# S-Taichiii/diffusion-model

Hardware: AMD Instinct MI355X
Metric: denoising steps/sec (CFG, T=1000, 32x32x4 latent, B=64) (higher is better)
Workload: dtype f32 (GEMMs: fp32 operands split fp16 hi+lo on the matrix cores, fp32 accumulate); 1 GPU; config 2: UnetCondWithGeomHead CFG=3.0 denoising step, B=64, 32x32x4, T=1000; global_batch=64, T=1000, parallelism=sample-sharded x1 (no per-step collective)

## Files before the change

### diffusion-model_amd/dmx/csrc/engine.hip

```cpp
#include "dmx.h"

#include <array>
#include <cmath>
#include <cstdio>
#include <cstdlib>
#include <cstring>
#include <functional>
#include <map>
#include <memory>
#include <stdexcept>
#include <string>
#include <vector>

#include "common.h"
#include "graph_slots.h"
#include "step_mode.h"
#include "igemm.h"
#include "igemm_x3.h"
#include "kernels.h"
#include "igemm_pp.h"
#include "launch.h"
#include "igemm_halo.h"
#include "tokmlp.h"
#include "eval.h"
// ... 953 lines not shown
  const bool a_scaled = a_scale.part != nullptr;
  const ConvPlan pl = conv_plan(R, cw, kind, N, H, W, epi, seg, a_scaled);
  const bool x3 = pl.x3, wino = pl.path == CONV_WINO;
  const int bm = pl.bm, bn = pl.bn, splits = pl.splits, x1 = pl.x1 ? 1 : 0;
  if (pl.path == CONV_INPUT) {
    if (res != nullptr) throw Error(DMX_E_INTERNAL, "gemm: the direct input conv takes no residual");
    if (ash != nullptr || asl != nullptr) throw Error(DMX_E_INTERNAL, "gemm: the direct input conv reads fp32 NCHW");
  } else if (a_scaled && (!x3 || ash != nullptr || epi == EPI_STATS || gn != nullptr || R.m->prec == 2)) {
    throw Error(DMX_E_INTERNAL, "gemm: device-scaled operands only on the plain split implicit GEMM");
  }
  if (gn != nullptr && ((pl.path != CONV_HALO && !wino) || ash != nullptr || src_mode != SRC_PLAIN))
    throw Error(DMX_E_INTERNAL, "gemm: GroupNorm-on-load needs the halo / Winograd conv on a plain fp32 source");
  float* partial = splits > 1 ? R.ws.get<float>((size_t)splits * M * cw.cout) : nullptr;
  if (defer != nullptr) {
    defer->fused = pl.fused;
    defer->partial = partial;
    defer->splits = splits;
    defer->bias = cw.bias;
  }
  if (R.plan) return pl.rrows;
  IgemmParams p;
  std::memset(&p, 0, sizeof(p));
  p.src = s;
  p.H = H;
  p.W = W;
  p.M = M;
  p.taps = cw.taps;
  p.geom = cw.phases == 4 ? 2 : (cw.taps == 9 ? 1 : (cw.taps == 16 ? 3 : 0));
  p.Hin = p.geom == 3 ? 2 * H : H;
  p.Win = p.geom == 3 ? 2 * W : W;
  p.Kreal = cw.taps * cw.cin;
  p.Kpad = cw.kpad;
  p.Cout = cw.cout;
  p.Npad = cw.npad;
  p.osy = p.osx = cw.phases == 4 ? 2 : 1;
  p.Hout = H * p.osy;
  p.Wout = W * p.osx;
  p.Bw = cw.B;
  p.bias = cw.bias;
  p.out = out;
  p.res = res;
  p.rowpart = rowpart;
  p.seg = seg;
  p.ksplit = pl.ksplit;
  p.partial = partial;
  p.rgrp = pl.rgrp;
  p.nphase = cw.phases;
  p.gexact = gelu_exact_flag(R);
  if (s.C != cw.cin) throw Error(DMX_E_INTERNAL, "gemm: source channels != weight channels");
  if (x3 && cw.cin < pl.bk) throw Error(DMX_E_INTERNAL, "gemm: x3 path needs Cin >= K-step");
  if (ash != nullptr && !x3) throw Error(DMX_E_INTERNAL, "gemm: f16-plane operand needs the split GEMM");
  if (src_mode != SRC_PLAIN && src_mode != SRC_NCHW) throw Error(DMX_E_INTERNAL, "gemm: unsupported source");
  const bool slabs_to_caller = splits > 1 && pl.fused && defer != nullptr;
  if (check_args()) {
    if (src_mode == SRC_PLAIN)
      check_range(R, s.src0, (size_t)N * p.Hin * p.Win * s.C * 4, "A");
    check_range(R, ash, (size_t)N * p.Hin * p.Win * s.C * 2, "A hi");
    check_range(R, asl, (size_t)N * p.Hin * p.Win * s.C * 2, "A lo");
    check_range(R, cw.B, (size_t)cw.phases * cw.npad * cw.kpad * 4, "B");
    check_range(R, partial, (size_t)splits * M * cw.cout * 4, "partial");
    if (!slabs_to_caller)
      check_range(R, out, (size_t)N * p.Hout * p.Wout * cw.cout * 4, "out");
    check_range(R, res, (size_t)N * p.Hout * p.Wout * cw.cout * 4, "res");
  }
  X3Params xp;
  xp.g = p;
  xp.Ash = ash;
  xp.Asl = asl;
  xp.Bh = cw.Bh;
  xp.Bl = cw.Bl;
  xp.inv_scale = cw.inv_scale;
  xp.Fh = cw.Fh;
  xp.Fl = cw.Fl;
  xp.gn_rowpart = nullptr;
  xp.gn_cnt = 0;
  xp.gn_gamma = xp.gn_beta = nullptr;
  xp.gn_res = nullptr;
  xp.Uh = xp.Ul = nullptr;
  xp.u_bytes = 0;
  xp.a_amax = a_scale.part;
  xp.a_nparts = a_scale.n;
  xp.w_inv = cw.inv_dev;
  {
    const size_t a_el = (size_t)N * p.Hin * p.Win * s.C;
    const size_t ab = a_el * (ash != nullptr ? 2 : 4), bb = (size_t)cw.npad * cw.kpad * 2;
    if (x3 && (ab >= ((size_t)1 << 31) || bb >= ((size_t)1 << 31)))
      throw Error(DMX_E_ARG, "gemm: operand too large for 32-bit buffer offsets (split the batch)");
    xp.a_bytes = (unsigned)ab;
    xp.b_bytes = (unsigned)bb;
  }
  const int gna = gn != nullptr ? (gn->res != nullptr ? 2 : 1) : 0;
  if (gna) {
    xp.gn_rowpart = gn->rowpart;
    xp.gn_cnt = gn->cnt;
    xp.gn_gamma = gn->gamma;
    xp.gn_beta = gn->beta;
    xp.gn_res = gn->res;
  }
  const int sa = ash != nullptr ? 1 : 0;
  const int creal = (src_mode == SRC_NCHW && s.C0) ? s.C0 : cw.cin;
  const double flops = 2.0 * (double)M * cw.phases * cw.cout * (double)cw.taps * creal;
  const double bytes = 4.0 * ((double)M * cw.phases * cw.cout + (double)N * p.Hin * p.Win * s.C +
                              (double)cw.phases * cw.cout * cw.taps * cw.cin) +
                       (splits > 1 ? 4.0 * splits * M * cw.cout : 0.0);
  const int e = splits > 1 ? (int)EPI_PARTIAL : epi;
  char nm[96];
  switch (pl.path) {
    case CONV_INPUT: {
      check_range(R, rowpart, (size_t)N * pl.rrows * (64 / 32) * sizeof(float2), "rowpart");
      ConvInParams q;
      q.x = s.src0;
      q.creal = s.C0 ? s.C0 : s.C;
      q.n_mod = s.n_mod;
      q.scale = s.scale;
      q.B = cw.B;
      q.cin = cw.cin;
      q.kpad = cw.kpad;
      q.out = out;
      q.rowpart = rowpart;
      q.H = H;
      q.W = W;
      R.begin(pl.cin_px == 32 ? "conv_in_kernel<32>" : "conv_in_kernel<16>", 2.0 * M * 64.0 * 9.0 * q.creal,
              4.0 * ((double)M * 64 + (double)M * q.creal));
      if (pl.cin_px == 32) conv_in_kernel<32><<<M / 32, 256, 0, R.st>>>(q);
      else conv_in_kernel<16><<<M / 16, 256, 0, R.st>>>(q);
      break;
    }
    case CONV_WINO:
      xp.Uh = cw.Uh;
      xp.Ul = cw.Ul;
      xp.u_bytes = (unsigned)((size_t)16 * cw.cout * s.C * 2);
      check_range(R, cw.Uh, xp.u_bytes, "U hi");
      check_range(R, cw.Ul, xp.u_bytes, "U lo");
      if (x1) std::snprintf(nm, sizeof nm, "wino_kernel<%d, %d, %d, 1>", pl.wg, gna, e);
      else std::snprintf(nm, sizeof nm, "wino_kernel<%d, %d, %d>", pl.wg, gna, e);
      R.begin(nm, flops, bytes);
      launch_wino(e, pl.wg, gna, x1, xp, dim3(wino_blocks(pl.wg, N, H), cw.cout / 64, splits), R.st);
// ... 20 lines not shown
        throw Error(DMX_E_INTERNAL, "bad epilogue");
      R.begin(nm, flops, bytes);
      if (e == EPI_PARTIAL) launch_x3_partial(bm, bn, sa, x1, xp, grid, R.st);
      else if (e == EPI_STATS) launch_x3_stats(bm, bn, sa, x1, xp, grid, R.st);
      else launch_x3_epi(e, bm, bn, sa, x1, xp, grid, R.st);
      break;
    }
    case CONV_F32: {
      const dim3 grid(cdiv(M, bm), cdiv(cw.cout, bn), splits > 1 ? splits : cw.phases);
      std::snprintf(nm, sizeof nm, "igemm_f32_kernel<%d, %d, %d, %d>", bm, bn, src_mode, e);
      if (src_mode == SRC_NCHW && e != EPI_PARTIAL && e != EPI_STATS)
        throw Error(DMX_E_INTERNAL, "bad epilogue for NCHW source");
      R.begin(nm, flops, bytes);
      launch_f32(src_mode, e, bm, bn, p, grid, R.st);
      break;
    }
  }
  R.end();
  HIPCHK(hipGetLastError());
  if (splits > 1 && !slabs_to_caller) splitk_reduce(R, pl, partial, M, cw, res, out, rowpart, seg, epi);
  return pl.rrows;
}

static void gn_finalize(Run& R, const float2* rowpart, float2* stats, int N, int rrows, int nseg, int G, int C,
                        int HWo) {
  if (R.plan) return;
  R.begin("gn_finalize_kernel", 0.0, 8.0 * (double)N * rrows * nseg);
  gn_finalize_kernel<<<N * G, 256, 0, R.st>>>(rowpart, stats, rrows, nseg, G, C, HWo, 1e-5f);
  R.end();
  HIPCHK(hipGetLastError());
}

static void norm(Run& R, NormParams np, int N) {
  if (R.plan) return;
  np.gexact = gelu_exact_flag(R);
  const int per = np.HW * (np.C / 4);
  const int target = 1024;
  const int chunks = std::max(1, std::min(cdiv(per, 256), std::max(cdiv(per, 1024), cdiv(target, N))));
  R.begin("norm_kernel", 0.0, 4.0 * (double)N * np.HW * np.C * (np.res ? 3 : 2));
  norm_kernel<<<dim3(chunks, N), 256, 0, R.st>>>(np);
  R.end();
  HIPCHK(hipGetLastError());
}

static void reduce_norm(Run& R, const Deferred& d, NormParams np, int n_src_samples) {
  if (R.plan) return;
  np.gexact = gelu_exact_flag(R);
  const int kv = std::max(RN_MIN_KV, cdiv(np.HW * (np.C / 4), 1024));
  const int n_out = np.n_src > 0 ? (np.n_fan > 0 ? np.n_fan : 2) * n_src_samples : n_src_samples;
  const int kvt = kv <= 2 ? 2 : kv <= 4 ? 4 : RN_MAXV;
  R.begin("reduce_norm_kernel<" + std::to_string(kvt) + ">", 0.0,
          4.0 * (double)n_src_samples * np.HW * np.C * (d.splits + (np.res ? 1 : 0)) +
              4.0 * (double)n_out * np.HW * np.C);
  if (kv <= 2) reduce_norm_kernel<2><<<n_src_samples, 1024, 0, R.st>>>(d.partial, d.splits, d.bias, np);
  else if (kv <= 4) reduce_norm_kernel<4><<<n_src_samples, 1024, 0, R.st>>>(d.partial, d.splits, d.bias, np);
  else reduce_norm_kernel<RN_MAXV><<<n_src_samples, 1024, 0, R.st>>>(d.partial, d.splits, d.bias, np);
  R.end();
  HIPCHK(hipGetLastError());
}

template <int SRC>
static void prep(Run& R, const SrcDesc& s, float* out, int N, int H, int W, const char* name, _Float16* oh = nullptr,
                 _Float16* ol = nullptr) {
  if (R.plan) return;
  const size_t total = (size_t)N * H * W * (s.C / 4);
  const int blocks = (int)std::min<size_t>((total + 255) / 256, 8192);
  R.begin(name, 0.0, 4.0 * (double)N * H * W * s.C * (SRC == SRC_MAXPOOL ? 5 : 2) * (oh ? 1.5 : 1.0));
  prep_kernel<SRC><<<blocks, 256, 0, R.st>>>(s, out, N, H, W, oh, ol);
  R.end();
  HIPCHK(hipGetLastError());
}

static SrcDesc plain_src(const float* p, int C) {
  SrcDesc s;
  std::memset(&s, 0, sizeof(s));
  s.src0 = p;
  s.C = C;
  s.G = 1;
  s.scale = 1.f;
  return s;
}

static NormParams norm_params(const float* raw, const float2* rowpart, int nseg, int rrows, const float* g,
                              const float* b, int C, int HW, float* out) {
  NormParams np;
  std::memset(&np, 0, sizeof(np));
  np.raw = raw;
  np.rowpart = rowpart;
  np.nseg = nseg;
  np.rrows = rrows;
  np.gamma = g;
  np.beta = b;
  np.C = C;
  np.G = 1;
  np.HW = HW;
  np.out = out;
  return np;
}

static float* resblock(Run& R, const ResW& w, const SrcDesc& in, int mode, int N, int H, int W, bool residual,
                       const float* emb, int emb_stride, int emb_off, int n_out = 0,
                       const _Float16* in_h = nullptr, const _Float16* in_l = nullptr, bool planes_out = false,
                       bool* wrote_planes = nullptr, GnLoad* defer_out = nullptr, const GnLoad* gn_in = nullptr) {
  const int M = N * H * W, HW = H * W;
  if (n_out <= 0) n_out = N;
  const int seg = 32;
  float* r1 = R.ws.get<float>((size_t)M * w.mid);
  float2* rp1 = R.ws.get<float2>((size_t)M * (w.mid / seg));
  const ConvPlan p2 = conv_plan(R, w.c2, CONV_SRC_PLAIN, N, H, W, EPI_STATS, seg);
  const bool planes = R.m->prec >= 1 && p2.takes_planes() && w.mid >= 64;
  float* a1 = R.ws.get<float>((size_t)M * w.mid);
  float* r2 = R.ws.get<float>((size_t)M * w.cout);
  float2* rp2 = R.ws.get<float2>((size_t)M * (w.cout / seg));
  float* out = R.ws.get<float>((size_t)n_out * HW * w.cout);
  Deferred d1, d2;
  if (gn_in != nullptr && (residual || mode != SRC_PLAIN))
    throw Error(DMX_E_INTERNAL, "resblock: a GroupNorm-on-load input needs a plain, non-residual block");
  const int rr1 = gemm(R, in, mode, N, H, W, w.c1, EPI_STATS, r1, nullptr, rp1, seg, in_h, in_l, &d1, gn_in);
  NormParams n1 = norm_params(r1, rp1, w.mid / seg, rr1, w.g1.p, w.b1.p, w.mid, HW, a1);
  n1.act = 1;
  _Float16* a1h = reinterpret_cast<_Float16*>(a1);
  _Float16* a1l = a1h + (size_t)M * w.mid;
  if (planes) {
    n1.out = nullptr;
    n1.out_h = a1h;
    n1.out_l = a1l;
  }
  const bool fuse1 = !d1.fused && !R.m->debug && p2.gn_load_pays(1) &&
                     (planes || p2.path == CONV_WINO);
  int rr2;
  if (fuse1) {
    GnLoad g;
    g.rowpart = rp1;
    g.cnt = rr1 * (w.mid / seg);
    g.gamma = w.g1.p;
    g.beta = w.b1.p;
    rr2 = gemm(R, plain_src(r1, w.mid), SRC_PLAIN, N, H, W, w.c2, EPI_STATS, r2, nullptr, rp2, seg, nullptr, nullptr,
               &d2, &g);
  } else {
    if (d1.fused) reduce_norm(R, d1, n1, N);
    else norm(R, n1, N);
    rr2 = gemm(R, plain_src(a1, w.mid), SRC_PLAIN, N, H, W, w.c2, EPI_STATS, r2, nullptr, rp2, seg,
               planes ? a1h : nullptr, planes ? a1l : nullptr, &d2);
  }
  if (defer_out != nullptr) *defer_out = GnLoad{};
  if (defer_out != nullptr && residual && mode == SRC_PLAIN && !d2.fused && emb == nullptr && n_out == N &&
      !R.m->debug) {
    defer_out->rowpart = rp2;
    defer_out->cnt = rr2 * (w.cout / seg);
    defer_out->gamma = w.g2.p;
    defer_out->beta = w.b2.p;
    defer_out->res = in.src0;
    if (wrote_planes != nullptr) *wrote_planes = false;
    return r2;
  }
  NormParams n2 = norm_params(r2, rp2, w.cout / seg, rr2, w.g2.p, w.b2.p, w.cout, HW, out);
  if (residual) {
    if (mode != SRC_PLAIN) throw Error(DMX_E_INTERNAL, "residual ResBlock needs a plain input");
    n2.res = in.src0;
  }
  n2.emb = emb;
  n2.emb_stride = emb_stride;
  n2.emb_off = emb_off;
  n2.n_src = n_out > N ? N : 0;
  n2.n_fan = n_out > N ? n_out / N : 0;
  const bool pout = planes_out && R.m->prec >= 1 && !R.m->debug && emb == nullptr && n_out == N && w.cout >= 64;
  if (wrote_planes != nullptr) *wrote_planes = pout;
  if (pout) {
    n2.out = nullptr;
    n2.out_h = reinterpret_cast<_Float16*>(out);
    n2.out_l = n2.out_h + (size_t)n_out * HW * w.cout;
  }
  if (d2.fused) reduce_norm(R, d2, n2, N);
  else norm(R, n2, n_out);
  R.tap(R.layer + ".r1", r1, (size_t)M * w.mid);
  R.tap(R.layer, out, (size_t)n_out * HW * w.cout);
  return out;
}

static void layernorm(Run& R, const float* x, float* y, const Vec& w, const Vec& b, int M, int C) {
  if (R.plan) return;
  const int blocks = cdiv(M, 4);
  R.begin("layernorm_kernel<" + std::to_string(C / 64) + ">", 0.0, 8.0 * (double)M * C);
  switch (C) {
    case 64: layernorm_kernel<1><<<blocks, 256, 0, R.st>>>(x, y, w.p, b.p, M, 1e-5f); break;
    case 128: layernorm_kernel<2><<<blocks, 256, 0, R.st>>>(x, y, w.p, b.p, M, 1e-5f); break;
    case 256: layernorm_kernel<4><<<blocks, 256, 0, R.st>>>(x, y, w.p, b.p, M, 1e-5f); break;
    default: throw Error(DMX_E_INTERNAL, "layernorm: unsupported C");
  }
  R.end();
  HIPCHK(hipGetLastError());
}

static void attention_core(Run& R, const float* qkv, float* out, int N, int L, int C, float* stats = nullptr) {
  if (R.plan) return;
  const int D = C / 4;
  if (D != 16 && D != 32 && D != 64) throw Error(DMX_E_INTERNAL, "attention: unsupported head dim");
  const bool x3 = R.m->prec >= 1 || stats != nullptr;
  if (stats != nullptr && R.m->prec == 2) throw Error(DMX_E_INTERNAL, "attention stats: not in fp16 mode");
  if (x3 && D == 16 && att16_lds_bytes(L, 0) <= 160 * 1024) {
    const int x1 = R.m->prec == 2 ? 1 : 0, nw = L > 256 ? 16 : 8;
    R.begin("attention16_kernel<" + std::to_string(nw) + ", " + std::to_string(x1) + ">", 4.0 * N * (double)L * L * C,
            4.0 * (double)N * L * 4 * C);
    HIPCHK(launch_attention16(nw, x1, qkv, out, L, C, N, R.st, stats));
    R.end();
    HIPCHK(hipGetLastError());
    return;
  }
  if (x3) {
    dim3 grid(cdiv(L, 128), 4, N);
    const int x1 = R.m->prec == 2 ? 1 : 0, wpe = D == 16 ? 4 : 1;
    R.begin("attention_x3_kernel<" + std::to_string(D) + ", " + std::to_string(wpe) + ", " + std::to_string(x1) + ">",
// ... 194 lines not shown
    SrcDesc mp = plain_src(cur, cc);
    mp.Hs = ch;
    mp.Ws = cw;
    const int nh = ch / 2, nw = cw / 2;
    const int nb = i == 0 ? S : N;
    R.layer = "down" + std::to_string(i + 1) + ".0";
    const size_t pool_el = (size_t)nb * nh * nw * cc;
    float* pooled = R.ws.get<float>(pool_el);
    const ConvPlan r0c1 = conv_plan(R, m->down[i].r0.c1, CONV_SRC_PLAIN, nb, nh, nw, EPI_STATS, 32);
    const ConvPlan r1c1 = conv_plan(R, m->down[i].r1.c1, CONV_SRC_PLAIN, nb, nh, nw, EPI_STATS, 32);
    const bool pool_planes = R.m->prec >= 1 && m->down[i].r0.c1.Bh != nullptr && !R.m->debug && !r0c1.reads_fp32();
    _Float16* pool_h = pool_planes ? R.ws.get<_Float16>(2 * pool_el) : nullptr;
    _Float16* pool_l = pool_planes ? pool_h + pool_el : nullptr;
    prep<SRC_MAXPOOL>(R, mp, pooled, nb, nh, nw, "prep_kernel<2>", pool_h, pool_l);
    bool hp = false;
    float* h0 = resblock(R, m->down[i].r0, plain_src(pooled, cc), SRC_PLAIN, nb, nh, nw, true, nullptr, 0, 0, 0,
                         pool_h, pool_l, r1c1.takes_planes(), &hp);
    R.layer = "down" + std::to_string(i + 1) + ".1";
    const _Float16* h0h = hp ? reinterpret_cast<const _Float16*>(h0) : nullptr;
    float* h1 = resblock(R, m->down[i].r1, plain_src(h0, cc), SRC_PLAIN, nb, nh, nw, false, emb, m->hsum,
                         m->down[i].emb_off, N, h0h, hp ? h0h + (size_t)nb * nh * nw * cc : nullptr);
    cc = m->down[i].cout;
    ch = nh;
    cw = nw;
    R.layer = "sa" + std::to_string(i + 1);
    cur = attn_block(R, m->sa[i], h1, N, ch, cw);
  }
  const _Float16 *cur_h = nullptr, *cur_l = nullptr;
  for (int i = 0; i < m->nbot; ++i) {
    R.layer = "bot" + std::to_string(i + 1);
    bool hp = false;
    const bool nxt = i + 1 < m->nbot &&
                     conv_plan(R, m->bot[i + 1].c1, CONV_SRC_PLAIN, N, ch, cw, EPI_STATS, 32).takes_planes();
    cur = resblock(R, m->bot[i], plain_src(cur, cc), SRC_PLAIN, N, ch, cw, false, nullptr, 0, 0, 0, cur_h, cur_l, nxt,
                   &hp);
    cc = m->bot[i].cout;
    cur_h = hp ? reinterpret_cast<const _Float16*>(cur) : nullptr;
    cur_l = hp ? cur_h + (size_t)N * ch * cw * cc : nullptr;
  }
  for (int i = 0; i < 3; ++i) {
    const int si = 2 - i;
    SrcDesc u = plain_src(skips[si], sc[si] + cc);
    u.C0 = sc[si];
    u.n_mod = si == 0 && S < N ? S : 0;
    u.src1 = cur;
    u.Hs = ch;
    u.Ws = cw;
    const int dy = sh[si] - 2 * ch, dx = sw[si] - 2 * cw;
    u.padT = dy > 0 ? dy / 2 : 0;
    u.padL = dx > 0 ? dx / 2 : 0;
    REQUIRE(u.C == m->up[i].r0.cin, "up: channel mismatch");
    R.layer = "up" + std::to_string(i + 1) + ".0";
    const size_t cat_el = (size_t)N * sh[si] * sw[si] * u.C;
    float* cat = R.ws.get<float>(cat_el);
    const ConvPlan r0c1 = conv_plan(R, m->up[i].r0.c1, CONV_SRC_PLAIN, N, sh[si], sw[si], EPI_STATS, 32);
    const ConvPlan r1c1 = conv_plan(R, m->up[i].r1.c1, CONV_SRC_PLAIN, N, sh[si], sw[si], EPI_STATS, 32);
    const bool cat_planes = R.m->prec >= 1 && m->up[i].r0.c1.Bh != nullptr && !R.m->debug && !r0c1.reads_fp32();
    _Float16* cat_h = cat_planes ? R.ws.get<_Float16>(2 * cat_el) : nullptr;
    _Float16* cat_l = cat_planes ? cat_h + cat_el : nullptr;
    prep<SRC_UPCAT>(R, u, cat, N, sh[si], sw[si], "prep_kernel<3>", cat_h, cat_l);
    bool hp = false;
    GnLoad dly;
    const bool try_defer = !R.m->debug && R.m->prec >= 1 && r1c1.gn_load_pays(2);
    float* h0 = resblock(R, m->up[i].r0, plain_src(cat, u.C), SRC_PLAIN, N, sh[si], sw[si], true, nullptr, 0, 0, 0,
                         cat_h, cat_l, r1c1.takes_planes(), &hp, try_defer ? &dly : nullptr);
    R.layer = "up" + std::to_string(i + 1) + ".1";
    const _Float16* h0h = hp ? reinterpret_cast<const _Float16*>(h0) : nullptr;
    float* h1 = dly.rowpart != nullptr
                    ? resblock(R, m->up[i].r1, plain_src(h0, u.C), SRC_PLAIN, N, sh[si], sw[si], false, emb, m->hsum,
                               m->up[i].emb_off, 0, nullptr, nullptr, false, nullptr, nullptr, &dly)
                    : resblock(R, m->up[i].r1, plain_src(h0, u.C), SRC_PLAIN, N, sh[si], sw[si], false, emb, m->hsum,
                               m->up[i].emb_off, 0, h0h, hp ? h0h + (size_t)N * sh[si] * sw[si] * u.C : nullptr);
    ch = sh[si];
    cw = sw[si];
    cc = m->up[i].cout;
    R.layer = "sa" + std::to_string(4 + i);
    cur = attn_block(R, m->sa[3 + i], h1, N, ch, cw);
  }
  return const_cast<float*>(cur);
}

static void check_shapes(dmx_model* m, int n, int h, int w) {
  if (!m->finalized) throw Error(DMX_E_STATE, "model weights not finalized");
  if (m->kind == DMX_VAE) throw Error(DMX_E_ARG, "not a U-Net model");
  REQUIRE(n >= 1, "batch must be >= 1");
  REQUIRE(h >= 8 && w >= 8, "latent must be at least 8x8");
  REQUIRE(h == w, "AttenionBlock assumes square maps (models/unet_cond.py:46-47)");
  REQUIRE(m->ctx->pos_table != nullptr, "time table not set (dmx_set_time_table)");
}

using GraphSlot = decltype(dmx_model::graphs)::Slot;

static void drop_slot(dmx_model* m, GraphSlot* s) {
  if (s->val.gexec) (void)hipGraphExecDestroy(s->val.gexec);
  if (s->val.graph) (void)hipGraphDestroy(s->val.graph);
  if (s->val.gexec_k) (void)hipGraphExecDestroy(s->val.gexec_k);
  if (s->val.graph_k) (void)hipGraphDestroy(s->val.graph_k);
  m->graphs.release(s);
}

static void drop_graph(dmx_model* m) {
  for (GraphSlot& s : m->graphs.slot) drop_slot(m, &s);
}

static void ensure_planes(dmx_model* m, hipStream_t st) {
  if (!m->planes_stale || m->prec < 1) return;
  drop_graph(m);
  for_each_conv(m, [&](ConvW& c) {
    if (c.Bh != nullptr) split_planes(c, st, m->amax);
  });
  m->planes_stale = false;
}

static bool poison_ws() {
  static const bool v = [] {
    const char* e = std::getenv("DMX_POISON");
    return e != nullptr && std::atoi(e) != 0;
  }();
// ... 835 lines not shown
```

### diffusion-model_amd/dmx/csrc/igemm_wino.h

```cpp
#pragma once
#include "common.h"
#include "igemm.h"
#include "igemm_x3.h"
#include "source.h"

namespace dmx {

#ifndef DMX_DIAG
#define DMX_DIAG 0
#endif
#if DMX_DIAG
constexpr int WSTAMP_SLOTS = 32, WSTAMP_BLOCKS = 2048;
__device__ unsigned long long g_wstamp[WSTAMP_SLOTS * WSTAMP_BLOCKS * 5];
DMX_DEV void wstamp(int slot, int k) {
  if (threadIdx.x == 0 && slot >= 0 && slot < WSTAMP_SLOTS) {
    const int b = (blockIdx.z * gridDim.y + blockIdx.y) * gridDim.x + blockIdx.x;
    if (b < WSTAMP_BLOCKS) {
      unsigned long long* q = g_wstamp + ((size_t)slot * WSTAMP_BLOCKS + b) * 5;
      q[k] = __builtin_amdgcn_s_memtime();
      if (k == 0) q[4] = ((unsigned long long)__builtin_amdgcn_s_getreg((20 << 0) | (0 << 6) | (3 << 11)) << 32) |
                         (unsigned)__builtin_amdgcn_s_getreg((4 << 0) | (0 << 6) | (31 << 11));
    }
  }
}
// ... 21 lines not shown
    const size_t f = q >> 6;
    const int kk = (int)(f % KK), nb = (int)((f / KK) % NB), xi = (int)(f / ((size_t)KK * NB));
    const int co = 32 * nb + (lane & 31), c0 = 16 * kk + 8 * (lane >> 5);
    half8 h, l;
#pragma unroll
    for (int e = 0; e < 8; ++e) {
      double g[3][3];
#pragma unroll
      for (int t = 0; t < 9; ++t) g[t / 3][t % 3] = (double)B[(size_t)co * kpad + (size_t)t * cin + c0 + e];
      const float u = (float)(wino_u(g, xi >> 2, xi & 3) * (double)scale);
      const _Float16 hh = (_Float16)u;
      h[e] = hh;
      l[e] = (_Float16)(u - (float)hh);
    }
    *reinterpret_cast<half8*>(uh + q * 8) = h;
    *reinterpret_cast<half8*>(ul + q * 8) = l;
  }
}

template <int W, int GNA, int EPI = EPI_STATS, int X1 = 0>
__global__ __launch_bounds__(512) void wino_kernel(const X3Params P) {
  static_assert(EPI == EPI_STATS || EPI == EPI_PARTIAL, "Winograd epilogues");
  static_assert(W == 32 || W == 16 || W == 8 || W == 4, "Winograd conv: image width 4, 8, 16 or 32");
  static_assert(W != 4 || GNA == 0, "W = 4: no GroupNorm-on-load instances");
  const IgemmParams& p = P.g;
  constexpr int TW = W / 2;
  constexpr int SPB = W == 8 ? 4 : W == 4 ? 16 : 1;
  constexpr int TPS = 64 / SPB;
  constexpr int HRS = (W == 32 ? 8 : W) + 2;
  constexpr int PS = W == 8 ? 11 : HRS;
  constexpr int HR = SPB * PS, HC = W + 2;
  constexpr int RP = W == 32 ? 88 : W == 16 ? 46 : W == 8 ? 26 : 18;
  constexpr int SQ = W == 4 ? 218 * 4 : PS * 8 * RP;
  constexpr int HBUF = SPB * SQ;
  constexpr bool RING0 = W == 4;
  constexpr int CK = 16;
  constexpr int NPC = RING0 ? SPB * W * W * (CK / 4) : HR * HC * (CK / 4);
  constexpr int NPI = (NPC + 511) / 512;
  static_assert(!RING0 || NPC % 512 == 0, "W = 4: interior pieces must fill whole thread rounds");
  constexpr int EPP = 34;
  constexpr int EPF = 16 * 32 * EPP;
  constexpr int LDSF = 2 * HBUF + 1024 > EPF ? 2 * HBUF + 1024 : EPF;
  __shared__ __attribute__((aligned(16))) float lds[LDSF];

  WSTAMP(0);
  const int tid = threadIdx.x, lane = tid & 63;
  const int wid = __builtin_amdgcn_readfirstlane(tid >> 6);
  const int wi = wid >> 1, jp = wid & 1;
  int mt, nt, bz;
  xcd_tile(mt, nt, bz);
  const int WA = p.W;
  const int BPS = W == 32 ? (p.H + 7) >> 3 : 1;
  const int HW = p.H * WA, C = p.src.C;
  const int nsmp = W == 32 ? mt / BPS : mt * SPB;
  const int band = W == 32 ? mt - nsmp * BPS : 0;
  const int y0 = 8 * band;
  const int nsamp = p.M / HW;
  const int nch_all = C / CK;
  const int cbeg = EPI == EPI_PARTIAL ? bz * p.ksplit : 0;
  const int nch = EPI == EPI_PARTIAL ? min(p.ksplit, nch_all - cbeg) : nch_all;

  int hoff[NPI], hls[NPI];
#pragma unroll
  for (int k = 0; k < NPI; ++k) {
    const int e = tid + 512 * k;
    const int h = e >> 2, q = e & 3;
    int hrow, hcol;
    if constexpr (RING0) {
      hrow = h / HC;
      hcol = h - hrow * HC;
    } else if constexpr (W == 32) {
      const int pr = (h >> 1) % 17, m = h & 1;
      hrow = (h >> 1) / 17;
      hcol = pr < 8 ? pr + 8 * m : pr < 16 ? 8 + pr + 8 * m : 32 + m;
    } else {
      const int t = (h >> 1) / HC;
      hcol = (h >> 1) - t * HC;
      hrow = 2 * t + (h & 1);
    }
    const int sh = RING0 ? h >> 4 : hrow / PS;
    const int ry = RING0 ? ((h >> 2) & 3) + 1 : hrow - sh * PS;
    const int hx = RING0 ? (h & 3) + 1 : hcol;
    const int y = y0 + ry - 1, x = hx - 1;
    const bool ok = e < NPC && ry < HRS && y >= 0 && y < p.H && x >= 0 && x < WA && nsmp + sh < nsamp;
    hoff[k] = ok ? ((((nsmp + sh) * p.H + y) * WA + x) * C + q * 4) : -1;
    hls[k] = e < NPC ? (sh * SQ + (ry * 2 + (hx & 1)) * RP * 4 + (hx >> 1) * 20 + q * 4) : 2 * HBUF + (tid & 255) * 4;
  }
  const __amdgpu_buffer_rsrc_t rA = rsrc_of(p.src.src0, P.a_bytes);
  const __amdgpu_buffer_rsrc_t rRes = rsrc_of(GNA == 2 ? (const void*)P.gn_res : (const void*)p.src.src0, P.a_bytes);

  __shared__ float2 gst_s[SPB];
  if constexpr (GNA) {
    __shared__ double gr1[4], gr2[4];
    for (int sp = 0; sp < SPB; ++sp) {
      if (tid < 256 && nsmp + sp < nsamp) {
        const float2* rp = P.gn_rowpart + (size_t)(nsmp + sp) * P.gn_cnt;
        double s1 = 0.0, s2 = 0.0;
        for (int i = tid; i < P.gn_cnt; i += 256) {
          const float2 q = rp[i];
          s1 += (double)q.x;
          s2 += (double)q.y;
        }
        s1 = wave_sum_dpp(s1);
        s2 = wave_sum_dpp(s2);
        if ((tid & 63) == 0) {
          gr1[tid >> 6] = s1;
          gr2[tid >> 6] = s2;
        }
      }
      __syncthreads();
      if (tid == 0) {
        const double cntd = (double)HW * (double)C;
        const double mean = ((gr1[0] + gr1[1]) + (gr1[2] + gr1[3])) / cntd;
        double var = ((gr2[0] + gr2[1]) + (gr2[2] + gr2[3])) / cntd - mean * mean;
        var = var < 0.0 ? 0.0 : var;
        gst_s[sp] = make_float2((float)mean, (float)(1.0 / sqrt(var + 1e-5)));
      }
      __syncthreads();
    }
  }

  floatx4 ha[NPI];
  floatx4 hr[GNA == 2 ? NPI : 1];
  auto load_halo = [&](int c) {
#pragma unroll
    for (int k = 0; k < NPI; ++k) {
      const int off = hoff[k] >= 0 ? (hoff[k] + (cbeg + c) * CK) * 4 : kOOB;
      ha[k] = bload_f4(rA, off, 0);
      if constexpr (GNA == 2) hr[k] = bload_f4(rRes, off, 0);
    }
  };
  auto store_halo = [&](int buf, int c) {
    float* hb = lds + buf * HBUF;
    floatx4 ggam = {0.f, 0.f, 0.f, 0.f}, gbet = {0.f, 0.f, 0.f, 0.f};
    if constexpr (GNA) {
      const int ch = (cbeg + c) * CK + (tid & 3) * 4;
      ggam = ld4(P.gn_gamma + ch);
      gbet = ld4(P.gn_beta + ch);
    }
#pragma unroll
    for (int k = 0; k < NPI; ++k) {
      floatx4 v = ha[k];
      if constexpr (GNA) {
        const float2 gst = gst_s[SPB == 1 ? 0 : min(hls[k] / SQ, SPB - 1)];
        v = gn_apply4v(v, gst, ggam, gbet, GNA == 1 ? 1 : 0);
        if constexpr (GNA == 2) {
#pragma unroll
          for (int j = 0; j < 4; ++j) v[j] = gelu(hr[k][j] + v[j]);
        }
        if (hoff[k] < 0) v = floatx4{0.f, 0.f, 0.f, 0.f};
      }
      *reinterpret_cast<floatx4*>(hb + hls[k]) = v;
    }
  };

  const int xi0 = 4 * wi + 2 * jp;
  const int NB = p.Cout / 32, KK = C / 16;
  const __amdgpu_buffer_rsrc_t rUh = rsrc_of(P.Uh, P.u_bytes), rUl = rsrc_of(P.Ul, P.u_bytes);
  int ub[2][2];
#pragma unroll
  for (int q = 0; q < 2; ++q)
#pragma unroll
    for (int n = 0; n < 2; ++n) ub[q][n] = (((xi0 + q) * NB + 2 * nt + n) * KK) * 1024;
  const int voff = lane * 16;
  half8 bh[2][2], bl[2][2];
  int cnext = 0;
  auto load_b = [&](int q, int n, int c) {
    const int cc = c < 0 ? cnext : c;
    bh[q][n] = bload_h8(rUh, voff, ub[q][n] + (cbeg + cc) * 1024);
    if constexpr (!X1) bl[q][n] = bload_h8(rUl, voff, ub[q][n] + (cbeg + cc) * 1024);
  };

  const int ra = wi == 0 ? 0 : wi == 2 ? 2 : 1;
  const int rb = wi == 0 ? 2 : wi == 2 ? 1 : wi == 1 ? 2 : 3;
  const float sr = wi == 1 ? 1.f : -1.f;
  const int cp = jp ? 2 : 0, cq = jp ? 1 : 2, cs = jp ? 3 : 1;
  const float sb = jp ? -1.f : 1.f;
  auto coff = [&](int col) { return (col & 1) * RP * 4 + (col >> 1) * 20; };
  const int oa = ra * 8 * RP, ob = rb * 8 * RP;
  const int op = coff(cp), oq = coff(cq), os = coff(cs);
  const int fr = lane & 31, fh = lane >> 5;
// ... 266 lines not shown
```

### diffusion-model_amd/dmx/csrc/kernels.h

```cpp
#pragma once
#include "common.h"
#include "source.h"
#include "tail_math.h"

namespace dmx {

DMX_DEV float wave_sum(float v) {
#pragma unroll
  for (int o = 32; o > 0; o >>= 1) v += __shfl_xor(v, o, 64);
  return v;
}

struct EmbedParams {
  const int64_t* t; int t_stride; int tmax;
  int t_mod;
  const int64_t* y;
  int y_null_first;
  int64_t y_null; int n_half;
  const float* vals; const float* mask;
  int cond_rows;
  const float* pos_table;
  const float* class_emb;
  int ncls;
  const float* w0; const float* b0;
// ... 143 lines not shown
    s2 += __shfl_xor(s2, off, 64);
  }
  if ((tid & 31) == 0) red[pg][co >> 5] = make_float2(s1, s2);
  __syncthreads();
  if (tid < 2)
    p.rowpart[((size_t)n * (HW / PX) + r / PX) * 2 + tid] =
        make_float2((red[0][tid].x + red[1][tid].x) + (red[2][tid].x + red[3][tid].x),
                    (red[0][tid].y + red[1][tid].y) + (red[2][tid].y + red[3][tid].y));
}

static __global__ __launch_bounds__(256) void gn_finalize_kernel(const float2* rowpart, float2* stats, int R, int nseg,
                                                           int G, int C, int HWo, float eps) {
  const int ng = blockIdx.x, n = ng / G, g = ng % G;
  const int spg = nseg / G;
  const int cnt = R * spg;
  double s1 = 0.0, s2 = 0.0;
  for (int i = threadIdx.x; i < cnt; i += 256) {
    const int r = i / spg, sg = g * spg + (i - r * spg);
    const float2 v = rowpart[((size_t)n * R + r) * nseg + sg];
    s1 += (double)v.x;
    s2 += (double)v.y;
  }
  __shared__ double r1[256], r2[256];
  r1[threadIdx.x] = s1;
  r2[threadIdx.x] = s2;
  __syncthreads();
  for (int o = 128; o > 0; o >>= 1) {
    if (threadIdx.x < o) {
      r1[threadIdx.x] += r1[threadIdx.x + o];
      r2[threadIdx.x] += r2[threadIdx.x + o];
    }
    __syncthreads();
  }
  if (threadIdx.x == 0) {
    const double cntd = (double)HWo * (double)(C / G);
    const double mean = r1[0] / cntd;
    double var = r2[0] / cntd - mean * mean;
    var = var < 0.0 ? 0.0 : var;
    stats[ng] = make_float2((float)mean, (float)(1.0 / sqrt(var + (double)eps)));
  }
}

struct NormParams {
  const float* raw; const float2* rowpart; int nseg; int rrows; const float2* stats;
  const float* gamma; const float* beta;
  int C, G, HW;
  const float* res; int act;
  int gexact;
  const float* emb; int emb_stride; int emb_off;
  int n_src;
  int n_fan;
  float* out;
  _Float16* out_h; _Float16* out_l;
};

DMX_DEV void st4(float* a, floatx4 v) { *reinterpret_cast<floatx4*>(a) = v; }
static __global__ __launch_bounds__(256) void norm_kernel(const NormParams p) {
  const int n = blockIdx.y, tid = threadIdx.x;
  const int ns = p.n_src > 0 ? n % p.n_src : n;
  const int C4 = p.C >> 2;
  const int per = p.HW * C4;
  const int chunk = (((per + (int)gridDim.x - 1) / (int)gridDim.x) + 255) & ~255;
  const int beg = blockIdx.x * chunk, end = min(per, beg + chunk);
  const size_t base = (size_t)n * per * 4, sbase = (size_t)ns * per * 4;
  const float* raw = p.raw + sbase;
  const float* res = p.res != nullptr ? p.res + sbase : nullptr;
  floatx4 v[4], r[4];
  auto load = [&](int i0) {
#pragma unroll
    for (int k = 0; k < 4; ++k) {
      const int idx = min(i0 + 256 * k, end - 1);
      v[k] = ld4(raw + (size_t)idx * 4);
      if (res != nullptr) r[k] = ld4(res + (size_t)idx * 4);
    }
  };
  int i0 = beg + tid;
  if (i0 < end) load(i0);
  const int cpg = p.C / p.G;
  const bool cfix = (256 % C4) == 0;
  const int cthr = (tid % C4) * 4;
  floatx4 fg{}, fb{}, fe{};
  if (cfix) {
    fg = ld4(p.gamma + cthr);
    fb = ld4(p.beta + cthr);
    if (p.emb != nullptr) fe = ld4(p.emb + (size_t)n * p.emb_stride + p.emb_off + cthr);
  }

  __shared__ double r1[4], r2[4];
  __shared__ float2 st_s;
  if (p.rowpart != nullptr) {
    const int cnt = p.rrows * p.nseg;
    const float2* rp = p.rowpart + (size_t)ns * cnt;
    double s1 = 0.0, s2 = 0.0;
    for (int i = tid; i < cnt; i += 256) {
      const float2 q = rp[i];
      s1 += (double)q.x;
      s2 += (double)q.y;
    }
    s1 = wave_sum_dpp(s1);
    s2 = wave_sum_dpp(s2);
    if ((tid & 63) == 0) {
      r1[tid >> 6] = s1;
      r2[tid >> 6] = s2;
    }
    __syncthreads();
    if (tid == 0) {
      const double cntd = (double)p.HW * (double)p.C;
      const double mean = ((r1[0] + r1[1]) + (r1[2] + r1[3])) / cntd;
      double var = ((r2[0] + r2[1]) + (r2[2] + r2[3])) / cntd - mean * mean;
      var = var < 0.0 ? 0.0 : var;
      st_s = make_float2((float)mean, (float)(1.0 / sqrt(var + 1e-5)));
    }
    __syncthreads();
  }
  for (; i0 < end; i0 += 1024) {
#pragma unroll
    for (int k = 0; k < 4; ++k) {
      const int idx = i0 + 256 * k;
      if (idx >= end) break;
      const int c = cfix ? cthr : (idx % C4) * 4;
      const float2 st = p.rowpart != nullptr ? st_s : p.stats[ns * p.G + c / cpg];
      floatx4 o = cfix ? gn_apply4v(v[k], st, fg, fb, 0) : gn_apply4(v[k], st, p.gamma, p.beta, c, 0);
      if (res != nullptr) {
        if (p.gexact) {
#pragma unroll
          for (int j = 0; j < 4; ++j) o[j] = gelu_exact(r[k][j] + o[j]);
        } else {
#pragma unroll
          for (int j = 0; j < 4; ++j) o[j] = gelu(r[k][j] + o[j]);
        }
      } else if (p.act) {
        if (p.gexact) {
#pragma unroll
          for (int j = 0; j < 4; ++j) o[j] = gelu_exact(o[j]);
        } else {
#pragma unroll
          for (int j = 0; j < 4; ++j) o[j] = gelu(o[j]);
        }
      }
      if (p.emb != nullptr) {
        const floatx4 e = cfix ? fe : ld4(p.emb + (size_t)n * p.emb_stride + p.emb_off + c);
#pragma unroll
        for (int j = 0; j < 4; ++j) o[j] += e[j];
      }
      const size_t off = base + (size_t)idx * 4;
      if (p.out != nullptr) st4(p.out + off, o);
      if (p.out_h != nullptr) {
        half4 hh, ll;
        split4(o, hh, ll);
        *reinterpret_cast<half4*>(p.out_h + off) = hh;
        *reinterpret_cast<half4*>(p.out_l + off) = ll;
      }
    }
    if (i0 + 1024 < end) load(i0 + 1024);
  }
}

constexpr int RN_MAXV = 8;

template <int KV>
__global__ __launch_bounds__(1024) void reduce_norm_kernel(const float* partial, int splits, const float* bias,
                                                           const NormParams p) {
  static_assert(KV >= 2, "reduce_norm_kernel: the KV = 1 instance is retired (engine.hip RN_MIN_KV)");
  constexpr int SB = KV >= 16 ? 1 : 16 / KV;
  const int s = blockIdx.x, tid = threadIdx.x;
  const int C4 = p.C >> 2, per = p.HW * C4;
  const size_t sstride = (size_t)gridDim.x * per * 4;
  const size_t sbase = (size_t)s * per * 4;
  floatx4 v[KV];
  float s1 = 0.f, s2 = 0.f;
#pragma unroll
  for (int k = 0; k < KV; ++k) v[k] = floatx4{0.f, 0.f, 0.f, 0.f};
  for (int sp0 = 0; sp0 < splits; sp0 += SB) {
    floatx4 a[SB][KV];
#pragma unroll
    for (int b = 0; b < SB; ++b)
#pragma unroll
      for (int k = 0; k < KV; ++k) {
        const int idx = tid + 1024 * k;
        a[b][k] = (sp0 + b < splits && idx < per) ? ld4(partial + (sp0 + b) * sstride + sbase + (size_t)idx * 4)
                                                  : floatx4{0.f, 0.f, 0.f, 0.f};
      }
#pragma unroll
    for (int b = 0; b < SB; ++b)
#pragma unroll
      for (int k = 0; k < KV; ++k)
#pragma unroll
        for (int j = 0; j < 4; ++j) v[k][j] += a[b][k][j];
  }
#pragma unroll
  for (int k = 0; k < KV; ++k) {
    const int idx = tid + 1024 * k;
    if (idx < per) {
      if (bias != nullptr) {
        const floatx4 b = ld4(bias + (idx % C4) * 4);
#pragma unroll
        for (int j = 0; j < 4; ++j) v[k][j] += b[j];
      }
#pragma unroll
      for (int j = 0; j < 4; ++j) {
        s1 += v[k][j];
        s2 += v[k][j] * v[k][j];
      }
    }
  }
  __shared__ double r1[16], r2[16];
  __shared__ float2 st_s;
  const double d1 = wave_sum_dpp((double)s1), d2 = wave_sum_dpp((double)s2);
  if ((tid & 63) == 0) {
    r1[tid >> 6] = d1;
    r2[tid >> 6] = d2;
  }
  __syncthreads();
  if (tid == 0) {
    double a1 = 0.0, a2 = 0.0;
    for (int w = 0; w < 16; ++w) {
      a1 += r1[w];
      a2 += r2[w];
    }
    const double cnt = (double)p.HW * (double)p.C;
    const double mean = a1 / cnt;
    double var = a2 / cnt - mean * mean;
    var = var < 0.0 ? 0.0 : var;
    st_s = make_float2((float)mean, (float)(1.0 / sqrt(var + 1e-5)));
  }
  __syncthreads();
  const float2 st = st_s;
  const int nout = p.n_src > 0 ? (p.n_fan > 0 ? p.n_fan : 2) : 1;
  for (int q = 0; q < nout; ++q) {
    const int n = s + q * (p.n_src > 0 ? p.n_src : 0);
    const size_t base = (size_t)n * per * 4;
#pragma unroll
    for (int k = 0; k < KV; ++k) {
      const int idx = tid + 1024 * k;
      if (idx >= per) break;
      const int c = (idx % C4) * 4;
      floatx4 o = gn_apply4(v[k], st, p.gamma, p.beta, c, 0);
      if (p.res != nullptr) {
        const floatx4 r = ld4(p.res + sbase + (size_t)idx * 4);
        if (p.gexact) {
#pragma unroll
          for (int j = 0; j < 4; ++j) o[j] = gelu_exact(r[j] + o[j]);
        } else {
#pragma unroll
          for (int j = 0; j < 4; ++j) o[j] = gelu(r[j] + o[j]);
        }
      } else if (p.act) {
        if (p.gexact) {
#pragma unroll
          for (int j = 0; j < 4; ++j) o[j] = gelu_exact(o[j]);
        } else {
#pragma unroll
          for (int j = 0; j < 4; ++j) o[j] = gelu(o[j]);
        }
      }
      if (p.emb != nullptr) {
        const floatx4 e = ld4(p.emb + (size_t)n * p.emb_stride + p.emb_off + c);
#pragma unroll
        for (int j = 0; j < 4; ++j) o[j] += e[j];
      }
      const size_t off = base + (size_t)idx * 4;
      if (p.out != nullptr) *reinterpret_cast<floatx4*>(p.out + off) = o;
      if (p.out_h != nullptr) {
        half4 hh, ll;
        split4(o, hh, ll);
        *reinterpret_cast<half4*>(p.out_h + off) = hh;
        *reinterpret_cast<half4*>(p.out_l + off) = ll;
      }
    }
  }
}

template <int SRC>
__global__ __launch_bounds__(256) void prep_kernel(const SrcDesc s, float* out, int N, int H, int W, _Float16* oh,
                                                   _Float16* ol) {
  const int C4 = s.C / 4;
  const size_t total = (size_t)N * H * W * C4;
  for (size_t i = (size_t)blockIdx.x * 256 + threadIdx.x; i < total; i += (size_t)gridDim.x * 256) {
    const int c = (int)(i % C4) * 4;
    const size_t pix = i / C4;
    const int n = (int)(pix / ((size_t)H * W));
    const int rr = (int)(pix - (size_t)n * H * W);
    const int y = rr / W, x = rr - y * W;
    const floatx4 v = load_src4<SRC>(s, n, y, x, c, H, W);
    st4(out + pix * s.C + c, v);
    if (oh != nullptr) {
      half4 hh, ll;
      split4(v, hh, ll);
      *reinterpret_cast<half4*>(oh + pix * s.C + c) = hh;
      *reinterpret_cast<half4*>(ol + pix * s.C + c) = ll;
    }
  }
// ... 597 lines not shown
```

Baseline: 486.1 CFG batch-steps/s (B=64 per GPU; 2 U-Net forwards + update each).

## Read up-block skip and upsampled halves directly instead of materializing the concat

In the decoder up blocks, the first ResBlock no longer gets an explicitly concatenated tensor (plus optional fp16 hi/lo planes). Only the upsampled half is prepared. The Winograd conv halo loader picks between the skip buffer and the upsampled buffer by channel offset, and the residual add in norm_kernel/reduce_norm_kernel reads from both parts. This removes writing and re-reading the full concat buffer, at the cost of giving up the fp16-plane input and deferred GroupNorm for that block and adding per-element address logic in the residual path.

```diff
diff --git a/diffusion-model_amd/dmx/csrc/engine.hip b/diffusion-model_amd/dmx/csrc/engine.hip
--- a/diffusion-model_amd/dmx/csrc/engine.hip
+++ b/diffusion-model_amd/dmx/csrc/engine.hip
@@ -1029,8 +1029,15 @@
   if (ash != nullptr && !x3) throw Error(DMX_E_INTERNAL, "gemm: f16-plane operand needs the split GEMM");
   if (src_mode != SRC_PLAIN && src_mode != SRC_NCHW) throw Error(DMX_E_INTERNAL, "gemm: unsupported source");
   const bool slabs_to_caller = splits > 1 && pl.fused && defer != nullptr;
+  const bool two_part = src_mode == SRC_PLAIN && s.C0 > 0;
+  if (two_part && (!wino || gn != nullptr || ash != nullptr || s.src1 == nullptr || 2 * s.C0 != s.C || s.C0 % 16 != 0 ||
+                   (s.n_mod != 0 && pl.wg != 32 && pl.wg != 16)))
+    throw Error(DMX_E_INTERNAL, "gemm: a two-part source needs the plain Winograd conv and equal halves");
   if (check_args()) {
-    if (src_mode == SRC_PLAIN)
+    if (two_part) {
+      check_range(R, s.src0, (size_t)(s.n_mod ? s.n_mod : N) * H * W * s.C0 * 4, "A part 0");
+      check_range(R, s.src1, (size_t)N * H * W * (s.C - s.C0) * 4, "A part 1");
+    } else if (src_mode == SRC_PLAIN)
       check_range(R, s.src0, (size_t)N * p.Hin * p.Win * s.C * 4, "A");
     check_range(R, ash, (size_t)N * p.Hin * p.Win * s.C * 2, "A hi");
     check_range(R, asl, (size_t)N * p.Hin * p.Win * s.C * 2, "A lo");
@@ -1059,7 +1066,7 @@
   xp.a_nparts = a_scale.n;
   xp.w_inv = cw.inv_dev;
   {
-    const size_t a_el = (size_t)N * p.Hin * p.Win * s.C;
+    const size_t a_el = (size_t)N * p.Hin * p.Win * (two_part ? s.C0 : s.C);
     const size_t ab = a_el * (ash != nullptr ? 2 : 4), bb = (size_t)cw.npad * cw.kpad * 2;
     if (x3 && (ab >= ((size_t)1 << 31) || bb >= ((size_t)1 << 31)))
       throw Error(DMX_E_ARG, "gemm: operand too large for 32-bit buffer offsets (split the batch)");
@@ -1186,7 +1193,11 @@
   R.begin("reduce_norm_kernel<" + std::to_string(kvt) + ">", 0.0,
           4.0 * (double)n_src_samples * np.HW * np.C * (d.splits + (np.res ? 1 : 0)) +
               4.0 * (double)n_out * np.HW * np.C);
-  if (kv <= 2) reduce_norm_kernel<2><<<n_src_samples, 1024, 0, R.st>>>(d.partial, d.splits, d.bias, np);
+  if (np.res1 != nullptr) {
+    if (kv <= 2) reduce_norm_kernel<2, true><<<n_src_samples, 1024, 0, R.st>>>(d.partial, d.splits, d.bias, np);
+    else if (kv <= 4) reduce_norm_kernel<4, true><<<n_src_samples, 1024, 0, R.st>>>(d.partial, d.splits, d.bias, np);
+    else reduce_norm_kernel<RN_MAXV, true><<<n_src_samples, 1024, 0, R.st>>>(d.partial, d.splits, d.bias, np);
+  } else if (kv <= 2) reduce_norm_kernel<2><<<n_src_samples, 1024, 0, R.st>>>(d.partial, d.splits, d.bias, np);
   else if (kv <= 4) reduce_norm_kernel<4><<<n_src_samples, 1024, 0, R.st>>>(d.partial, d.splits, d.bias, np);
   else reduce_norm_kernel<RN_MAXV><<<n_src_samples, 1024, 0, R.st>>>(d.partial, d.splits, d.bias, np);
   R.end();
@@ -1199,7 +1210,10 @@
   if (R.plan) return;
   const size_t total = (size_t)N * H * W * (s.C / 4);
   const int blocks = (int)std::min<size_t>((total + 255) / 256, 8192);
-  R.begin(name, 0.0, 4.0 * (double)N * H * W * s.C * (SRC == SRC_MAXPOOL ? 5 : 2) * (oh ? 1.5 : 1.0));
+  const double px = (double)N * H * W;
+  const double bytes = SRC == SRC_UPCAT ? 4.0 * (px * s.C * (oh ? 2.0 : 1.0) + px * s.C0 + (double)N * s.Hs * s.Ws * (s.C - s.C0))
+                                        : 4.0 * px * s.C * (SRC == SRC_MAXPOOL ? 5 : 2) * (oh ? 1.5 : 1.0);
+  R.begin(name, 0.0, bytes);
   prep_kernel<SRC><<<blocks, 256, 0, R.st>>>(s, out, N, H, W, oh, ol);
   R.end();
   HIPCHK(hipGetLastError());
@@ -1250,6 +1264,8 @@
   Deferred d1, d2;
   if (gn_in != nullptr && (residual || mode != SRC_PLAIN))
     throw Error(DMX_E_INTERNAL, "resblock: a GroupNorm-on-load input needs a plain, non-residual block");
+  if (mode == SRC_PLAIN && in.C0 > 0 && (defer_out != nullptr || in_h != nullptr))
+    throw Error(DMX_E_INTERNAL, "resblock: a two-part input is neither deferred nor read as planes");
   const int rr1 = gemm(R, in, mode, N, H, W, w.c1, EPI_STATS, r1, nullptr, rp1, seg, in_h, in_l, &d1, gn_in);
   NormParams n1 = norm_params(r1, rp1, w.mid / seg, rr1, w.g1.p, w.b1.p, w.mid, HW, a1);
   n1.act = 1;
@@ -1292,6 +1308,11 @@
   if (residual) {
     if (mode != SRC_PLAIN) throw Error(DMX_E_INTERNAL, "residual ResBlock needs a plain input");
     n2.res = in.src0;
+    if (in.C0 > 0) {
+      n2.res1 = in.src1;
+      n2.res_c0 = in.C0;
+      n2.res_nmod = in.n_mod;
+    }
   }
   n2.emb = emb;
   n2.emb_stride = emb_stride;
@@ -1592,18 +1613,38 @@
     REQUIRE(u.C == m->up[i].r0.cin, "up: channel mismatch");
     R.layer = "up" + std::to_string(i + 1) + ".0";
     const size_t cat_el = (size_t)N * sh[si] * sw[si] * u.C;
-    float* cat = R.ws.get<float>(cat_el);
     const ConvPlan r0c1 = conv_plan(R, m->up[i].r0.c1, CONV_SRC_PLAIN, N, sh[si], sw[si], EPI_STATS, 32);
+    const ConvPlan r0c2 = conv_plan(R, m->up[i].r0.c2, CONV_SRC_PLAIN, N, sh[si], sw[si], EPI_STATS, 32);
     const ConvPlan r1c1 = conv_plan(R, m->up[i].r1.c1, CONV_SRC_PLAIN, N, sh[si], sw[si], EPI_STATS, 32);
-    const bool cat_planes = R.m->prec >= 1 && m->up[i].r0.c1.Bh != nullptr && !R.m->debug && !r0c1.reads_fp32();
-    _Float16* cat_h = cat_planes ? R.ws.get<_Float16>(2 * cat_el) : nullptr;
-    _Float16* cat_l = cat_planes ? cat_h + cat_el : nullptr;
-    prep<SRC_UPCAT>(R, u, cat, N, sh[si], sw[si], "prep_kernel<3>", cat_h, cat_l);
-    bool hp = false;
     GnLoad dly;
     const bool try_defer = !R.m->debug && R.m->prec >= 1 && r1c1.gn_load_pays(2);
-    float* h0 = resblock(R, m->up[i].r0, plain_src(cat, u.C), SRC_PLAIN, N, sh[si], sw[si], true, nullptr, 0, 0, 0,
-                         cat_h, cat_l, r1c1.takes_planes(), &hp, try_defer ? &dly : nullptr);
+    const bool inplace = r0c1.path == CONV_WINO && 2 * u.C0 == u.C && u.C0 % 16 == 0 && !R.m->debug &&
+                         !(try_defer && !r0c2.fused) && (u.n_mod == 0 || r0c1.wg == 32 || r0c1.wg == 16);
+    bool hp = false;
+    float* h0;
+    if (inplace) {
+      SrcDesc up = u;
+      up.src0 = nullptr;
+      up.C = u.C - u.C0;
+      up.C0 = 0;
+      up.n_mod = 0;
+      float* upm = R.ws.get<float>(cat_el / 2);
+      prep<SRC_UPCAT>(R, up, upm, N, sh[si], sw[si], "prep_kernel<3>");
+      SrcDesc two = plain_src(skips[si], u.C);
+      two.src1 = upm;
+      two.C0 = u.C0;
+      two.n_mod = u.n_mod;
+      h0 = resblock(R, m->up[i].r0, two, SRC_PLAIN, N, sh[si], sw[si], true, nullptr, 0, 0, 0, nullptr, nullptr,
+                    r1c1.takes_planes(), &hp, nullptr);
+    } else {
+      float* cat = R.ws.get<float>(cat_el);
+      const bool cat_planes = R.m->prec >= 1 && m->up[i].r0.c1.Bh != nullptr && !R.m->debug && !r0c1.reads_fp32();
+      _Float16* cat_h = cat_planes ? R.ws.get<_Float16>(2 * cat_el) : nullptr;
+      _Float16* cat_l = cat_planes ? cat_h + cat_el : nullptr;
+      prep<SRC_UPCAT>(R, u, cat, N, sh[si], sw[si], "prep_kernel<3>", cat_h, cat_l);
+      h0 = resblock(R, m->up[i].r0, plain_src(cat, u.C), SRC_PLAIN, N, sh[si], sw[si], true, nullptr, 0, 0, 0,
+                    cat_h, cat_l, r1c1.takes_planes(), &hp, try_defer ? &dly : nullptr);
+    }
     R.layer = "up" + std::to_string(i + 1) + ".1";
     const _Float16* h0h = hp ? reinterpret_cast<const _Float16*>(h0) : nullptr;
     float* h1 = dly.rowpart != nullptr
diff --git a/diffusion-model_amd/dmx/csrc/igemm_wino.h b/diffusion-model_amd/dmx/csrc/igemm_wino.h
--- a/diffusion-model_amd/dmx/csrc/igemm_wino.h
+++ b/diffusion-model_amd/dmx/csrc/igemm_wino.h
@@ -97,6 +97,7 @@
   const int WA = p.W;
   const int BPS = W == 32 ? (p.H + 7) >> 3 : 1;
   const int HW = p.H * WA, C = p.src.C;
+  const int CS = GNA == 0 && p.src.C0 > 0 ? p.src.C0 : C, CP = CS;
   const int nsmp = W == 32 ? mt / BPS : mt * SPB;
   const int band = W == 32 ? mt - nsmp * BPS : 0;
   const int y0 = 8 * band;
@@ -128,10 +129,13 @@
     const int hx = RING0 ? (h & 3) + 1 : hcol;
     const int y = y0 + ry - 1, x = hx - 1;
     const bool ok = e < NPC && ry < HRS && y >= 0 && y < p.H && x >= 0 && x < WA && nsmp + sh < nsamp;
-    hoff[k] = ok ? ((((nsmp + sh) * p.H + y) * WA + x) * C + q * 4) : -1;
+    hoff[k] = ok ? ((((nsmp + sh) * p.H + y) * WA + x) * CP + q * 4) : -1;
     hls[k] = e < NPC ? (sh * SQ + (ry * 2 + (hx & 1)) * RP * 4 + (hx >> 1) * 20 + q * 4) : 2 * HBUF + (tid & 255) * 4;
   }
-  const __amdgpu_buffer_rsrc_t rA = rsrc_of(p.src.src0, P.a_bytes);
+  const float* a0 = p.src.src0;
+  if (GNA == 0 && p.src.n_mod) a0 += ((ptrdiff_t)(nsmp % p.src.n_mod) - nsmp) * (ptrdiff_t)HW * CP;
+  const __amdgpu_buffer_rsrc_t rA = rsrc_of(GNA == 0 ? a0 : p.src.src0, P.a_bytes);
+  const __amdgpu_buffer_rsrc_t rA1 = rsrc_of(GNA == 0 ? p.src.src1 : p.src.src0, P.a_bytes);
   const __amdgpu_buffer_rsrc_t rRes = rsrc_of(GNA == 2 ? (const void*)P.gn_res : (const void*)p.src.src0, P.a_bytes);
 
   __shared__ float2 gst_s[SPB];
@@ -168,10 +172,13 @@
   floatx4 ha[NPI];
   floatx4 hr[GNA == 2 ? NPI : 1];
   auto load_halo = [&](int c) {
+    const bool part1 = GNA == 0 && (cbeg + c) * CK >= CS;
+    const int cb = (cbeg + c) * CK - (part1 ? CS : 0);
+    const __amdgpu_buffer_rsrc_t r = part1 ? rA1 : rA;
 #pragma unroll
     for (int k = 0; k < NPI; ++k) {
-      const int off = hoff[k] >= 0 ? (hoff[k] + (cbeg + c) * CK) * 4 : kOOB;
-      ha[k] = bload_f4(rA, off, 0);
+      const int off = hoff[k] >= 0 ? (hoff[k] + cb) * 4 : kOOB;
+      ha[k] = bload_f4(r, off, 0);
       if constexpr (GNA == 2) hr[k] = bload_f4(rRes, off, 0);
     }
   };
diff --git a/diffusion-model_amd/dmx/csrc/kernels.h b/diffusion-model_amd/dmx/csrc/kernels.h
--- a/diffusion-model_amd/dmx/csrc/kernels.h
+++ b/diffusion-model_amd/dmx/csrc/kernels.h
@@ -219,7 +219,17 @@
   int n_fan;
   float* out;
   _Float16* out_h; _Float16* out_l;
+  const float* res1; int res_c0; int res_nmod;
 };
+
+DMX_DEV const float* res_part4(const NormParams& p, int ns, int pix, int c4) {
+  const int q0 = p.res_c0 >> 2;
+  if (c4 < q0) {
+    const int n0 = p.res_nmod ? ns % p.res_nmod : ns;
+    return p.res + ((size_t)n0 * p.HW + pix) * p.res_c0 + c4 * 4;
+  }
+  return p.res1 + ((size_t)ns * p.HW + pix) * (p.C - p.res_c0) + (c4 - q0) * 4;
+}
 
 DMX_DEV void st4(float* a, floatx4 v) { *reinterpret_cast<floatx4*>(a) = v; }
 static __global__ __launch_bounds__(256) void norm_kernel(const NormParams p) {
@@ -231,21 +241,35 @@
   const int beg = blockIdx.x * chunk, end = min(per, beg + chunk);
   const size_t base = (size_t)n * per * 4, sbase = (size_t)ns * per * 4;
   const float* raw = p.raw + sbase;
-  const float* res = p.res != nullptr ? p.res + sbase : nullptr;
+  const bool res2 = p.res1 != nullptr;
+  const float* res = p.res != nullptr ? p.res + (res2 ? 0 : sbase) : nullptr;
+  const int cpg = p.C / p.G;
+  const bool cfix = (256 % C4) == 0;
+  const int cthr = (tid % C4) * 4;
+  const float* rfix = nullptr;
+  int rpitch = 0, c4sh = 0;
+  if (res2 && cfix) {
+    rfix = res_part4(p, ns, 0, cthr >> 2);
+    rpitch = cthr < p.res_c0 ? p.res_c0 : p.C - p.res_c0;
+    c4sh = 31 - __clz(C4);
+  }
+  auto res_at = [&](int idx) -> const float* {
+    if (!res2) return res + (size_t)idx * 4;
+    if (cfix) return rfix + (size_t)(idx >> c4sh) * rpitch;
+    const int pix = idx / C4;
+    return res_part4(p, ns, pix, idx - pix * C4);
+  };
   floatx4 v[4], r[4];
   auto load = [&](int i0) {
 #pragma unroll
     for (int k = 0; k < 4; ++k) {
       const int idx = min(i0 + 256 * k, end - 1);
       v[k] = ld4(raw + (size_t)idx * 4);
-      if (res != nullptr) r[k] = ld4(res + (size_t)idx * 4);
+      if (res != nullptr) r[k] = ld4(res_at(idx));
     }
   };
   int i0 = beg + tid;
   if (i0 < end) load(i0);
-  const int cpg = p.C / p.G;
-  const bool cfix = (256 % C4) == 0;
-  const int cthr = (tid % C4) * 4;
   floatx4 fg{}, fb{}, fe{};
   if (cfix) {
     fg = ld4(p.gamma + cthr);
@@ -325,7 +349,7 @@
 
 constexpr int RN_MAXV = 8;
 
-template <int KV>
+template <int KV, bool RES2 = false>
 __global__ __launch_bounds__(1024) void reduce_norm_kernel(const float* partial, int splits, const float* bias,
                                                            const NormParams p) {
   static_assert(KV >= 2, "reduce_norm_kernel: the KV = 1 instance is retired (engine.hip RN_MIN_KV)");
@@ -404,7 +428,9 @@
       const int c = (idx % C4) * 4;
       floatx4 o = gn_apply4(v[k], st, p.gamma, p.beta, c, 0);
       if (p.res != nullptr) {
-        const floatx4 r = ld4(p.res + sbase + (size_t)idx * 4);
+        const float* rq = p.res + sbase + (size_t)idx * 4;
+        if constexpr (RES2) rq = res_part4(p, s, idx / C4, idx % C4);
+        const floatx4 r = ld4(rq);
         if (p.gexact) {
 #pragma unroll
           for (int j = 0; j < 4; ++j) o[j] = gelu_exact(r[j] + o[j]);
```

New measurement: 489.0 CFG batch-steps/s (B=64 per GPU; 2 U-Net forwards + update each), median of 6. No clear change (+0.6%).
